# AbbVie-ComputationalGenomics/SAIGEgds

Measured on AMD Instinct MI355X. Metric: variants/sec seqAssocGLMM_SPA at N=430K; achieved HBM GB/s vs roofline, higher is better.
Workload: dtype f64

## Files before the change

saigegds_amd/csrc/host_init.h:

```cpp
extern "C" const char *sgx_version(void) { return "saigehip 0.1 (gfx950)"; }
extern "C" const char *sgx_last_error(void) { return g_err.c_str(); }

extern "C" int sgx_device_count(void)
{
	int n = 0;
	if (hipGetDeviceCount(&n) != hipSuccess) return 0;
	return n;
}

extern "C" size_t sgx_row_stride(int32_t n_samp)
{
	return (size_t)((n_samp + 511) / 512) * 128;
}

static double thr_or(double v, double dflt) { return std::isfinite(v) ? v : dflt; }

extern "C" int sgx_set_thresholds(sgx_handle *h, double maf, double mac, double missing,
	double spa_pval)
{
	if (!h) return fail(SGX_EINVAL, "sgx_set_thresholds: NULL handle");
	h->md.thr_maf = thr_or(maf, -1);
	h->md.thr_mac = thr_or(mac, -1);
	h->md.thr_missing = thr_or(missing, 1);
	h->md.thr_spa = thr_or(spa_pval, 0.05);
// ... 63 lines not shown
		}
	}
	if (!(worst <= 1e-13L * scale)) return false;
	for (int a = 0; a < K; a++)
		for (int b = 0; b < K; b++) out[(size_t)b * K + a] = (double)M[(size_t)a * K + b];
	for (int a = 0; a < K * K; a++) if (!std::isfinite(out[a])) return false;
	return true;
}

static int alloc_workspace(sgx_handle *h)
{
	const int N = h->md.N;
	{
		int least = 0, greatest = 0;
		HIPCHK(hipDeviceGetStreamPriorityRange(&least, &greatest));
		HIPCHK(hipStreamCreateWithPriority(&h->stream, hipStreamNonBlocking, least));
		HIPCHK(hipStreamCreateWithPriority(&h->hstream, hipStreamNonBlocking, greatest));
		HIPCHK(hipStreamCreateWithPriority(&h->s3_side, hipStreamNonBlocking, greatest));
	}
	HIPCHK(hipEventCreateWithFlags(&h->s3_fork, hipEventDisableTiming));
	HIPCHK(hipEventCreateWithFlags(&h->s3_join, hipEventDisableTiming));
	HIPCHK(hipMalloc((void **)&h->counters, 24 * sizeof(int)));
	HIPCHK(hipHostMalloc((void **)&h->h_counters, 24 * sizeof(int), hipHostMallocDefault));
	for (int i = 0; i < 3; i++) HIPCHK(hipEventCreate(&h->ev[i]));
	for (int i = 0; i < 2; i++) HIPCHK(hipEventCreate(&h->evk[i]));
	HIPCHK(hipEventCreate(&h->ev_lists));
	hipDeviceProp_t prop;
	HIPCHK(hipGetDeviceProperties(&prop, h->device));
	h->spa_grid = prop.multiProcessorCount * 2;
	h->n_cu = prop.multiProcessorCount;
	h->scratch_stride = 2 * (((size_t)N + 63) & ~(size_t)63);
	HIPCHK(hipMalloc((void **)&h->scratch, h->scratch_stride * sizeof(double) * h->spa_grid));
	if (!h->md.quant) {
		h->nwg5 = ((size_t)((N + 63) / 64) * 16 <= 32 * 1024) ? h->n_cu * 4 : h->n_cu;
		HIPCHK(hipMalloc((void **)&h->scr5, (size_t)h->nwg5 * spa5_wg_bytes(N)));
		HIPCHK(hipMalloc((void **)&h->cur5, 8 * sizeof(int)));
	}
	return SGX_OK;
}

static int check_model_consistency(const sgx_model *m)
{
	const int N = m->n_samp, K = m->n_coeff;
	if (!m->t_XXVX_inv || !m->XV)
		return fail(SGX_EINVAL, "sgx_init: SAIGEHIP_CHECK_MODEL needs t_XXVX_inv and XV");
	for (int i = 0; i < N; i++) {
		const double *x = m->t_X + (size_t)i * K, *xv = m->XV + (size_t)i * K,
			*a = m->t_XXVX_inv + (size_t)i * K, *av = m->t_XVX_inv_XV + (size_t)i * K;
		int k0 = 0;
		double sx = 0, sa = 0;
		for (int k = 0; k < K; k++) {
			if (std::fabs(x[k]) > std::fabs(x[k0])) k0 = k;
			sx = std::max(sx, std::fabs(xv[k])); sa = std::max(sa, std::fabs(av[k]));
		}
		if (x[k0] == 0) continue;
		const double V = xv[k0] / x[k0];
		for (int k = 0; k < K; k++) {
			if (std::fabs(xv[k] - V * x[k]) > 1e-8 * sx)
				return fail(SGX_EINVAL, "sgx_init: XV[%d,%d] = %g is not V t_X = %g", k, i, xv[k], V * x[k]);
			if (std::fabs(av[k] - V * a[k]) > 1e-8 * sa)
				return fail(SGX_EINVAL, "sgx_init: t_XVX_inv_XV[%d,%d] = %g is not V t_XXVX_inv = %g",
					k, i, av[k], V * a[k]);
		}
	}
	return SGX_OK;
}

extern "C" int sgx_init(const sgx_model *m, int device, sgx_handle **out)
// ... 155 lines not shown
		TRY(dev_upload(&h->dFl, Flu));
		h->mf[0].Fl = h->dFl;
		TRY(dev_upload(&h->dQ, Qt));
	}
	md.F = h->dF; md.X = h->dX; md.y = h->dy; md.mu = h->dmu; md.mu2 = h->dmu2; md.XM = h->dXM;
	rc = alloc_workspace(h);
	if (rc) { sgx_free(h); return rc; }
#undef TRY
	*out = h;
	return SGX_OK;
}

extern "C" int sgx_score_layout(sgx_handle *h, int32_t *limbs, int32_t n_limbs, int32_t *n_groups)
{
	if (!h || !n_groups) return fail(SGX_EINVAL, "sgx_score_layout: NULL argument");
	*n_groups = h->mf_ok ? h->mfe.ngroups : 0;
	for (int c = 0; limbs && c < n_limbs; c++) limbs[c] = (h->mf_ok && c < h->md.P) ? h->mfe.climb[c] : 0;
	return SGX_OK;
}

extern "C" void sgx_free(sgx_handle *h)
{
	if (!h) return;
	(void)hipSetDevice(h->device);
	if (h->stream) (void)hipStreamSynchronize(h->stream);
	for (sgx_handle *&t : h->twins) if (t) { sgx_free(t); t = nullptr; }
	if (!h->shares_model) {
		(void)hipFree(h->dF); (void)hipFree(h->dX); (void)hipFree(h->dy);
		(void)hipFree(h->dmu); (void)hipFree(h->dmu2); (void)hipFree(h->dXM); (void)hipFree(h->dFl); (void)hipFree(h->dQ);
	}
	(void)hipFree(h->fallback); (void)hipFree(h->fb_spa2); (void)hipFree(h->fb_x2);
	(void)hipFree(h->s3_slabs); (void)hipFree(h->s3_t3); (void)hipFree(h->s3_ovf);
	for (int b = 0; b < 2; b++) if (h->tmp_blk[b]) { sgx_block_free(h->tmp_blk[b]); h->tmp_blk[b] = nullptr; }
	(void)hipFree(h->mf_acc); (void)hipFree(h->seg4); (void)hipFree(h->scr5); (void)hipFree(h->cur5);
	(void)hipFree(h->recs); (void)hipFree(h->counters); (void)hipFree(h->scratch);
	for (int b = 0; b < 2; b++) {
		(void)hipFree(h->pipe_in[b]); (void)hipFree(h->pipe_pk[b]); (void)hipFree(h->pipe_raw[b]); (void)hipFree(h->pipe_out[b]); (void)hipFree(h->pipe_valid[b]);
		if (h->pin_out[b]) (void)hipHostFree(h->pin_out[b]);
		if (h->pin_valid[b]) (void)hipHostFree(h->pin_valid[b]);
	}
	(void)hipFree(h->pipe_flag); (void)hipFree(h->pk_sel);
	if (h->h_pipe_flag) (void)hipHostFree(h->h_pipe_flag);
	if (h->ev_h2d) (void)hipEventDestroy(h->ev_h2d);
	for (int k = 0; k < 2; k++) { if (h->ev_copy[k]) (void)hipEventDestroy(h->ev_copy[k]); if (h->ev_done[k]) (void)hipEventDestroy(h->ev_done[k]); }
	if (h->cstream) (void)hipStreamDestroy(h->cstream);
	(void)hipFree(h->stage_in); (void)hipFree(h->stage_out); (void)hipFree(h->stage_valid); (void)hipFree(h->stage_pk); (void)hipFree(h->ds_part);
	if (h->h_counters) (void)hipHostFree(h->h_counters);
	for (int i = 0; i < 3; i++) if (h->ev[i]) (void)hipEventDestroy(h->ev[i]);
	for (int i = 0; i < 2; i++) if (h->evk[i]) (void)hipEventDestroy(h->evk[i]);
	if (h->ev_lists) (void)hipEventDestroy(h->ev_lists);
	if (h->s3_side) { (void)hipStreamSynchronize(h->s3_side); (void)hipStreamDestroy(h->s3_side); }
	if (h->hstream) { (void)hipStreamSynchronize(h->hstream); (void)hipStreamDestroy(h->hstream); }
	if (h->s3_fork) (void)hipEventDestroy(h->s3_fork);
	if (h->s3_join) (void)hipEventDestroy(h->s3_join);
	if (h->stream) (void)hipStreamDestroy(h->stream);
	delete h;
}

static int ensure_recs(sgx_handle *h, size_t n)
{
	if (n <= h->recs_cap) return SGX_OK;
	HIPCHK(hipStreamSynchronize(h->stream));
	if (h->recs) HIPCHK(hipFree(h->recs));
	if (h->fallback) HIPCHK(hipFree(h->fallback));
	h->recs = nullptr; h->fallback = nullptr; h->recs_cap = 0;
	HIPCHK(hipMalloc((void **)&h->recs, 3 * n * sizeof(SpaRec)));
	HIPCHK(hipMalloc((void **)&h->fallback, n * sizeof(int)));
// ... 23 lines not shown
```

saigegds_amd/csrc/host_lanes.h:

```cpp
extern "C" int sgx_set_option(sgx_handle *h, const char *name, long long value)
{
	if (!h || !name) return fail(SGX_EINVAL, "sgx_set_option: NULL argument");
	const std::string n(name);
	if (n == "score_v1") h->force_v1 = value != 0;
	else if (n == "force_dense") h->force_dense = value != 0;
	else if (n == "spa_exact") h->force_exact = value != 0;
	else if (n == "pipe_mb") { if (value < 0 || value > 65536) return fail(SGX_EINVAL, "pipe_mb out of range"); h->pipe_bytes = (size_t)value << 20; return SGX_OK; }
	else if (n == "spa_abl") h->spa_abl = (int)value;
	else if (n == "guard_exp") { if (value < 0 || value > 300) return fail(SGX_EINVAL, "guard_exp must be 0..300"); h->guard_tol = std::pow(10.0, -(double)value); }
	else if (n == "three_plane") { if (value < -1 || value > 1) return fail(SGX_EINVAL, "three_plane must be -1 (automatic), 0 or 1"); h->dense_opt = (int)value; return SGX_OK; }
	else if (n == "lanes") {
		if (value < 1 || value > 4) return fail(SGX_EINVAL, "lanes must be 1..4");
		if (h->owner) return fail(SGX_EINVAL, "lanes: not on a twin");
		int rc = sgx_sync(h);
		if (rc) return rc;
		for (int i = (int)value - 1; i < 3; i++) if (h->twins[i]) { sgx_free(h->twins[i]); h->twins[i] = nullptr; }
		for (int i = 0; i < (int)value - 1; i++) {
			if (h->twins[i]) continue;
			sgx_handle *t = new sgx_handle();
			t->device = h->device; t->md = h->md; t->mf_ok = h->mf_ok; t->mfe = h->mfe;
			for (int g = 0; g < MF_MAXG; g++) { t->mf[g] = h->mf[g]; t->mf_nbfv[g] = h->mf_nbfv[g]; }
			t->dF = h->dF; t->dX = h->dX; t->dy = h->dy; t->dmu = h->dmu; t->dmu2 = h->dmu2; t->dXM = h->dXM; t->dFl = h->dFl; t->dQ = h->dQ;
			t->shares_model = true; t->owner = h;
			t->force_dense = h->force_dense; t->force_v1 = h->force_v1; t->force_exact = h->force_exact;
// ... 8 lines not shown
	}
	else return fail(SGX_EINVAL, "sgx_set_option: unknown option '%s'", name);
	for (sgx_handle *t : h->twins) if (t) { int rc = sgx_set_option(t, name, value); if (rc) return rc; }
	return SGX_OK;
}

static void stats_add(sgx_stats &into, const sgx_stats &x)
{
	into.n_variants += x.n_variants; into.n_valid += x.n_valid; into.n_spa += x.n_spa;
	into.n_spa_dense += x.n_spa_dense; into.n_spa_slow += x.n_spa_slow;
	into.ms_score += x.ms_score; into.ms_spa += x.ms_spa; into.ms_total += x.ms_total;
	into.ms_kernel += x.ms_kernel; into.ms_lists += x.ms_lists;
	into.score_launches += x.score_launches; into.spa_launches += x.spa_launches;
	into.three_plane += x.three_plane; into.n_unlisted += x.n_unlisted; into.n_guarded += x.n_guarded;
}

static int sync_lane(sgx_handle *h)
{
	int rc = set_dev(h);
	if (rc) return rc;
	HIPCHK(hipStreamSynchronize(h->stream));
	if (h->pend_dense.active) {
		h->pend_dense.active = false;
		if (h->stats_pending && h->h_counters[2] > 0) {
			rc = launch_pending_dense(h);
			if (rc) return rc;
			HIPCHK(hipStreamSynchronize(h->stream));
		}
	}
	if (h->stats_pending) {
		h->stats.n_spa = (uint64_t)(h->h_counters[0] + h->h_counters[7] - h->h_counters[6] + h->h_counters[5]);
		h->stats.n_valid = (uint64_t)h->h_counters[1];
		h->stats.n_spa_dense = (uint64_t)h->h_counters[2];
		h->stats.n_spa_slow = (uint64_t)h->h_counters[4];
		h->stats.three_plane = h->form == FORM_THREE ? 1u : 0u;
		h->stats.n_guarded = (uint32_t)h->h_counters[21];
		h->stats.n_unlisted = (uint32_t)h->h_counters[23] - h->stats.n_guarded;
		if (h->form != FORM_FP64) {
			sgx_handle *p = h->owner ? h->owner : h;
			const double frac = 64.0 * (double)h->h_counters[22] / ((double)std::max<uint64_t>(1, h->stats.n_variants) * (double)h->md.N);
			const bool over = (uint64_t)h->stats.n_unlisted * 32 > h->stats.n_variants;
			if (h->form != FORM_THREE && (frac > SGX_DENSE_ON || over)) p->dense_mode = true;
			else if (h->form == FORM_THREE && frac < SGX_DENSE_OFF) p->dense_mode = false;
		}
#ifdef SPA5_PROF
		fprintf(stderr, "routing: tier A %d, tier B %d (of them handed on by A: %d), per-variant kernels %d (series list %d, exact list %d), dense %d\n",
			h->h_counters[0], h->h_counters[7], h->h_counters[6], h->h_counters[5], h->h_counters[3], h->h_counters[4], h->h_counters[2]);
		fprintf(stderr, "spa5 phases (10 ns ticks summed over variants): series kernel %d variants: stage %d count %d index %d gather %d series %d (sweep %d sum %d solve %d) | exact kernel %d variants: stage %d count %d index %d gather %d - sweeps %d\n",
			h->h_counters[3], h->h_counters[8], h->h_counters[9], h->h_counters[10], h->h_counters[11], h->h_counters[12], h->h_counters[13], h->h_counters[14], h->h_counters[15],
			h->h_counters[4], h->h_counters[16], h->h_counters[17], h->h_counters[18], h->h_counters[19], h->h_counters[21]);
#endif
		float a = 0, b = 0, c = 0;
		(void)hipEventElapsedTime(&a, h->ev[0], h->ev[1]);
		(void)hipEventElapsedTime(&b, h->ev[1], h->ev[2]);
		(void)hipEventElapsedTime(&c, h->ev[0], h->ev[2]);
		h->stats.ms_score = a; h->stats.ms_spa = b; h->stats.ms_total = c;
		float k = 0;
		if (h->evk_set) (void)hipEventElapsedTime(&k, h->evk[0], h->evk[1]);
		h->stats.ms_kernel = k; h->evk_set = false;
		float l = 0;
		if (h->lists_timed) { (void)hipEventElapsedTime(&l, h->ev_lists, h->ev[0]); h->stats.ms_total += l; }
		h->stats.ms_lists = l; h->lists_timed = false;
		h->stats_pending = false;
		sgx_handle *p = h->owner ? h->owner : h;
		stats_add(p->total, h->stats);
		p->total_calls++;
	}
// ... 31 lines not shown
```

saigegds_amd/csrc/host_spa.h:

```cpp


template <int LO, typename F, int... I>
static bool with_int(int v, F &&f, std::integer_sequence<int, I...>)
{
	return ((v == LO + I && (f(std::integral_constant<int, LO + I>()), true)) || ...);
}
template <typename F>
static bool with_k(int K, F &&f) { return with_int<1>(K, f, std::make_integer_sequence<int, KMAX>()); }
template <typename F>
static void with_pp(int P, F &&f)
{
	if (P <= 8) f(std::integral_constant<int, 8>());
	else if (P <= 16) f(std::integral_constant<int, 16>());
	else if (P <= 32) f(std::integral_constant<int, 32>());
	else f(std::integral_constant<int, 64>());
}

static dim3 mf_grid(int n_cu, size_t rows, int ntile, int *tps, int vpb = MF_VPB, int wg_per_cu = 2)
{
	const int vt = (int)((rows + vpb - 1) / vpb);
	int sk = std::max(1, (n_cu * wg_per_cu * 4 + vt / 2) / vt);
	sk = std::min(sk, std::max(1, ntile / 24));
	if (sk >= 6) sk = (sk + 7) & ~7;
	sk = std::min(sk, std::max(1, ntile / 2));
// ... 1 lines not shown
	*tps += *tps & 1;
	sk = (ntile + *tps - 1) / *tps;
	return dim3((unsigned)vt, (unsigned)sk);
}

template <int KK, int NCX, int INPUT>
static const void *spa4_moments_fn()
{
	if constexpr (INPUT == IN_2BIT) return (const void *)spa4_moments<KK, NCX>;
	else return (const void *)spa4_moments_ds<KK, NCX, INPUT>;
}

template <int KK, int INPUT>
static int launch_spa_k(sgx_handle *h, RowsRef rr, size_t M, double *out8, bool lazy_dense)
{
	const DevModel &md = h->md;
	constexpr int PB = 512;
	hipStream_t st = h->stream;
	const dim3 sgrid((unsigned)std::min<size_t>(M, (size_t)h->spa_grid));
	if (h->force_v1 && INPUT != IN_2BIT) {
		hipLaunchKernelGGL((spa_kernel<KK, PB, INPUT>), sgrid, dim3(PB), 0, st, rr,
			md, h->recs, h->counters, 0, (const int *)nullptr, h->scratch, h->scratch_stride, out8);
		return SGX_OK;
	}
	const size_t fl = spa4_lds_bytes(KK);
	if (!h->mom_attr_set[INPUT]) {
		HIPCHK(hipFuncSetAttribute(spa4_moments_fn<KK, SPA4_NCA, INPUT>(), hipFuncAttributeMaxDynamicSharedMemorySize, (int)fl));
		HIPCHK(hipFuncSetAttribute(spa4_moments_fn<KK, SPA4_NCB, INPUT>(), hipFuncAttributeMaxDynamicSharedMemorySize, (int)fl));
		h->mom_attr_set[INPUT] = true;
	}
	const int nround = (int)((M + h->vcap4 - 1) / h->vcap4);
	const int btop = (int)(2 * M);
	const dim3 gsolve((unsigned)std::min((h->vcap4 + 3) / 4, 4 * h->n_cu));
	const size_t rowb5 = (size_t)((md.N + 63) / 64) * 16;
	const size_t l5 = (INPUT == IN_2BIT && rowb5 <= 120 * 1024) ? rowb5 : 0;
	const bool small5 = INPUT == IN_2BIT && rowb5 <= 32 * 1024;
	if (l5 > 48 * 1024 && !h->spa5_attr_set[INPUT]) {
		HIPCHK(hipFuncSetAttribute((const void *)spa5_kernel<KK, INPUT, 0, 512>, hipFuncAttributeMaxDynamicSharedMemorySize, (int)l5));
		HIPCHK(hipFuncSetAttribute((const void *)spa5_kernel<KK, INPUT, 1, 512>, hipFuncAttributeMaxDynamicSharedMemorySize, (int)l5));
		h->spa5_attr_set[INPUT] = true;
	}
	const int fx5 = (h->force_exact ? 1 : 0) | (h->spa_abl & ~1);
	auto moments = [&](auto ncx, int tier, int rd) {
		constexpr int NCX = decltype(ncx)::value;
		if constexpr (INPUT == IN_2BIT)
			hipLaunchKernelGGL((spa4_moments<KK, NCX>), dim3((unsigned)h->n_cu), dim3(WAVE * spa4_waves(KK)), fl, st, rr, md, h->nseg,
				tier, btop, rd * h->vcap4, h->vcap4, h->recs, h->counters, h->seg4, h->spa_abl, h->cur5 + 2);
		else
			hipLaunchKernelGGL((spa4_moments_ds<KK, NCX, INPUT>), dim3((unsigned)h->n_cu), dim3(WAVE * spa4_waves(KK)), fl, st,
				(const void *)rr.base, rr.bpv, md, h->nseg, tier, btop, rd * h->vcap4, h->vcap4, h->recs, h->counters, h->seg4, h->cur5 + 2);
		hipLaunchKernelGGL((spa4_solve<KK, NCX>), gsolve, dim3(256), 0, st, md, h->nseg, tier, btop, rd * h->vcap4, h->vcap4,
			h->recs, h->counters, h->seg4, h->fallback, h->fb_x2, out8, h->force_dense ? 1 : 0, h->force_exact ? 1 : 0);
	};
	for (int rd = 0; rd < nround; rd++) moments(std::integral_constant<int, SPA4_NCA>(), 0, rd);
	for (int rd = 0; rd < nround; rd++) moments(std::integral_constant<int, SPA4_NCB>(), 1, rd);
	const int only5 = (INPUT == IN_2BIT && rr.cptr != nullptr && (h->spa_abl & 512)) ? 2 : 0;
	const size_t ws5 = spa5_wg_bytes(md.N);
	auto spa5 = [&](auto threads, int nwg) {
		constexpr int T5 = decltype(threads)::value;
		if constexpr (T5 == 512 || INPUT == IN_2BIT) {
			hipLaunchKernelGGL((spa5_kernel<KK, INPUT, 0, T5>), dim3((unsigned)nwg), dim3(T5), l5, st, rr, md, h->recs, h->counters,
				h->fb_spa2, h->fb_x2, h->cur5, h->fallback, h->scr5, out8, h->force_dense ? 1 : 0, fx5, l5, only5, ws5, 3);
			hipLaunchKernelGGL((spa5_kernel<KK, INPUT, 1, T5>), dim3((unsigned)nwg), dim3(T5), l5, st, rr, md, h->recs, h->counters,
				h->fb_x2, h->fb_x2, h->cur5 + 1, h->fallback, h->scr5, out8, h->force_dense ? 1 : 0, fx5, l5, only5, ws5, 4);
		}
	};
	if (small5) spa5(std::integral_constant<int, 128>(), h->nwg5);
	else spa5(std::integral_constant<int, 512>(), h->n_cu);
	if (!lazy_dense)
		hipLaunchKernelGGL((spa_kernel<KK, PB, INPUT>), sgrid, dim3(PB), 0, st, rr,
			md, h->recs, h->counters, 2, h->fallback, h->scratch, h->scratch_stride, out8);
	return SGX_OK;
}

template <int INPUT>
static int launch_spa(sgx_handle *h, RowsRef rr, size_t M, double *out8, bool lazy_dense = false)
{
	h->stats.spa_launches = 0;
	if (h->md.quant) return SGX_OK;
	int rc = SGX_OK;
	with_k(h->md.K, [&](auto kk) { rc = launch_spa_k<decltype(kk)::value, INPUT>(h, rr, M, out8, lazy_dense); });
	if (rc) return rc;
	HIPCHK(hipGetLastError());
	const bool v1 = h->force_v1 && INPUT != IN_2BIT;
	h->stats.spa_launches = v1 ? 1u : (uint32_t)(4 * ((M + h->vcap4 - 1) / h->vcap4) + 3);
	if (lazy_dense && !v1) { h->pend_dense.active = true; h->pend_dense.rr = rr; h->pend_dense.M = M; h->pend_dense.out8 = out8; }
	return SGX_OK;
}

static int launch_pending_dense(sgx_handle *h)
{
	const dim3 sgrid((unsigned)std::min<size_t>(h->pend_dense.M, (size_t)h->spa_grid));
	with_k(h->md.K, [&](auto kk) {
		hipLaunchKernelGGL((spa_kernel<decltype(kk)::value, 512, IN_2BIT>), sgrid, dim3(512), 0, h->stream, h->pend_dense.rr, h->md,
			h->recs, h->counters, 2, h->fallback, h->scratch, h->scratch_stride, h->pend_dense.out8);
	});
	HIPCHK(hipGetLastError());
	return SGX_OK;
}

static int scan_begin(sgx_handle *h, hipStream_t sst, ScanForm form, const sgx_block *b)
// ... 84 lines not shown
```

saigegds_amd/csrc/host_state.h:

```cpp

struct sgx_block {
	int device = 0;
	int N = 0, ntile = 0, nr = 1;
	size_t cap = 0;
	size_t M = 0;
	bool lists_only = false;
	uint8_t *rows = nullptr;
	size_t bpv = 0;
	const uint8_t *ext_rows = nullptr; size_t ext_bpv = 0;
	unsigned *idx = nullptr; size_t idx_cap = 0;
	unsigned *cursor = nullptr;
	unsigned *lstart = nullptr;
	int *lcnt = nullptr;
	int *nzp = nullptr, *n2p = nullptr;
	int *n3 = nullptr;
	uint8_t *ovf = nullptr;
	int *nzv = nullptr, *n2v = nullptr;
	unsigned *cptr = nullptr;
	unsigned *cidx = nullptr;
	size_t cidx_cap = 0;
	uint8_t *corient = nullptr;
	hipEvent_t ready = nullptr;
	hipEvent_t last_read = nullptr;
	bool was_read = false;
	int *info = nullptr, *h_info = nullptr;
	bool info_read = false, dense = false;
};

enum ScanForm {
	FORM_FP64,
	FORM_LISTS,
	FORM_ROWS,
	FORM_THREE,
};

struct sgx_handle {
	int device = 0;
	hipStream_t stream = nullptr;
	DevModel md{};
	double *dF = nullptr, *dX = nullptr, *dy = nullptr, *dmu = nullptr, *dmu2 = nullptr, *dXM = nullptr;
	SpaRec *recs = nullptr; size_t recs_cap = 0;
	int *fallback = nullptr;
	int *fb_spa2 = nullptr;
	int *fb_x2 = nullptr;
	int nseg = 0;
	bool force_dense = false;
	double *seg4 = nullptr;
	int vcap4 = 0, nround4 = 0;
	bool spa5_attr_set[3] = {false, false, false};
	bool mom_attr_set[3] = {false, false, false};
	uint8_t *scr5 = nullptr; int *cur5 = nullptr; int nwg5 = 0;
	int spa_abl = 0;
	bool force_exact = false;
	bool mf_ok = false;
	MfTab mf[MF_MAXG]{};
	int mf_nbfv[MF_MAXG]{};
	MfEpi mfe{};
	uint8_t *dFl = nullptr;
	long long *dQ = nullptr;
	int *mf_acc = nullptr;
	int *s3_slabs = nullptr; size_t s3_slabs_cap = 0;
	long long *s3_t3 = nullptr; size_t s3_t3_cap = 0;
	int *s3_ovf = nullptr; size_t s3_ovf_cap = 0;
	bool s3_attr[17] = {false};
	bool s3_attr_miss[17] = {false};
	hipStream_t hstream = nullptr;
	hipStream_t s3_side = nullptr;
	hipEvent_t s3_fork = nullptr, s3_join = nullptr;
	sgx_block *tmp_blk[2] = {nullptr, nullptr};
	int n_cu = 256;
	int *counters = nullptr;
	int *h_counters = nullptr;
	double *scratch = nullptr; size_t scratch_stride = 0; int spa_grid = 0;
	uint8_t *stage_in = nullptr; size_t stage_in_cap = 0;
	hipStream_t cstream = nullptr;
	size_t pipe_bytes = 0;
	uint8_t *pipe_in[2] = {nullptr, nullptr}; size_t pipe_in_cap = 0;
	uint8_t *pipe_pk[2] = {nullptr, nullptr}; size_t pipe_pk_cap = 0;
	uint8_t *pipe_raw[2] = {nullptr, nullptr}; size_t pipe_raw_cap = 0;
	int *pk_sel = nullptr; size_t pk_sel_cap = 0;
	double *pipe_out[2] = {nullptr, nullptr}; uint8_t *pipe_valid[2] = {nullptr, nullptr}; size_t pipe_out_cap = 0;
	double *pin_out[2] = {nullptr, nullptr}; uint8_t *pin_valid[2] = {nullptr, nullptr};
	int *pipe_flag = nullptr, *h_pipe_flag = nullptr;
	hipEvent_t ev_h2d = nullptr;
// ... 36 lines not shown
```

saigegds_amd/csrc/kern_spa4.h:

```cpp
#pragma once
#include "kern_spa4_tab.h"


#ifndef SPA4_WAVES_LOWK
#define SPA4_WAVES_LOWK 8
#endif
__host__ __device__ constexpr int spa4_waves(int K) { return K <= 8 ? SPA4_WAVES_LOWK : 8; }
#define SPA4_NCA 12
#define SPA4_NCB SPA4_NC
#define SPA4_NSMAX (SPA4_NC + 5)
#define SPA4_TAIL_TOL 1e-10

__device__ __forceinline__ double spa4_fma_svv(double a_sgpr, double x, double c_vgpr)
{
	double r;
	asm("v_fma_f64 %0, %1, %2, %3" : "=v"(r) : "s"(a_sgpr), "v"(x), "v"(c_vgpr));
	return r;
}

__device__ __forceinline__ void spa4_max_abs(double &g, double a)
{
	asm("v_max_f64 %0, %0, |%1|" : "+v"(g) : "v"(a));
}

// ... 508 lines not shown
			recs[btop - 1 - slot] = r;
		} else {
			fb_exact[atomicAdd(&counters[4], 1)] = ri;
		}
		return;
	}
	double pval;
	bool converged = true;
	if ((st_mine & 2) && (st_other & 2)) {
		pval = fabs(p_mine) + fabs(p_other);
		if (pval != 0 && pn_in / pval > 1000) pval = pn_in;
	} else {
		pval = pn_in;
		converged = false;
	}
	spa_write_row(r, Tstat, var1, pval, converged, out8);
}


#define SPA5_BIG 2048

__device__ __forceinline__ void cgf_terms_rt(double g, double m, double t, bool with_k, double &k1, double &k2, double &k0)
{
	const double om = 1 - m, mg = m * g, c2 = om * mg * g;
	const double e = fast_exp(-g * t);
	const double d = fma(om, e, m);
	const double rr = isfinite(d) ? fast_rcp(d) : 0.0;
	k1 = fma(mg, rr, k1);
	const double tt = c2 * e * rr * rr;
	if (isfinite(tt)) k2 += tt;
	if (with_k) k0 += cgf_korg_term(g, m, t, d, om);
}

__host__ __device__ inline size_t spa5_wg_bytes(int N) { return (((size_t)N + 63) & ~(size_t)63) * (16 + 4); }

template <int BLOCK>
__device__ __noinline__ void spa5_cum_sweep(const double2 *__restrict__ glist, int nnz, double ts, double *kp_out)
{
	constexpr int NC = SPA4_NCB;
	double kp[NC - 1];
#pragma unroll
	for (int a = 0; a < NC - 1; a++) kp[a] = 0;
	double2 gn = (int)threadIdx.x < nnz ? glist[threadIdx.x] : make_double2(0.0, 0.5);
	for (int k = threadIdx.x; k < nnz; k += BLOCK) {
		const double2 gm = gn;
		if (k + BLOCK < nnz) gn = glist[k + BLOCK];
		const double mui = gm.y;
		spa4_cum_terms<NC>(gm.x * ts, mui * (1 - mui), 1 - 2 * mui, kp);
		kp[NC - 2] = fmax(kp[NC - 2], fabs(gm.x));
	}
#pragma unroll
	for (int a = 0; a < NC - 1; a++) kp_out[a] = kp[a];
}

__device__ __noinline__ int spa5_series_solve(const double *arg, const SpaRec *__restrict__ rec, double *__restrict__ out8)
{
	constexpr int NC = SPA4_NCB;
	Spa4Series<NC> S;
#pragma unroll
	for (int a = 0; a < NC - 2; a++) S.kp[a] = arg[a];
	S.k1 = arg[NC - 2]; S.k2 = arg[NC - 1]; S.ts = arg[NC]; S.gmax = arg[NC + 1];
	const double xmax = arg[NC + 2], qtilde = arg[NC + 3], qinv = arg[NC + 4], NAmu = arg[NC + 5], NAsigma = arg[NC + 6];
	const double pn_in = arg[NC + 7], Tstat = arg[NC + 8], var1 = arg[NC + 9];
	RootState s1, s2;
	if (!spa4_root(S, xmax, qtilde, NAmu, NAsigma, s1) || !spa4_root(S, xmax, qinv, NAmu, NAsigma, s2)) return 0;
	double pval;
	bool converged = true;
// ... 31 lines not shown
	const int lane = threadIdx.x & (WAVE - 1), wv = threadIdx.x / WAVE;
	double kr[NC - 2];
#pragma unroll
	for (int a = 0; a < NC - 2; a++) kr[a] = kp[a];
	const int idx = wave_reduce_scatter(kr, lane);
#pragma unroll
	for (int o = 32; o > 0; o >>= 1) gmax = fmax(gmax, __shfl_xor(gmax, o, WAVE));
	double *part = sh + NC + 16;
	if (!(lane & 3) && idx < NC - 2) part[idx * NWV + wv] = kr[0];
	if (lane == 1) part[(NC - 2) * NWV + wv] = gmax;
	__syncthreads();
	double *arg = sh;
	if (threadIdx.x < NC - 2) {
		double t = 0;
		for (int w = 0; w < NWV; w++) t += part[threadIdx.x * NWV + w];
		arg[threadIdx.x] = t;
	}
	__syncthreads();
	SPA5_TS(1);
	if (threadIdx.x == 0) {
		for (int w = 0; w < NWV; w++) gmax = fmax(gmax, part[(NC - 2) * NWV + w]);
		arg[NC - 2] = k1; arg[NC - 1] = k2; arg[NC] = ts; arg[NC + 1] = gmax; arg[NC + 2] = xmax;
		arg[NC + 3] = qtilde; arg[NC + 4] = qinv; arg[NC + 5] = NAmu; arg[NC + 6] = NAsigma;
		arg[NC + 7] = pn_in; arg[NC + 8] = Tstat; arg[NC + 9] = var1;
		*sh_flag = spa5_series_solve(arg, rec, out8);
	}
	SPA5_TS(2);
	__syncthreads();
	const bool done = *sh_flag != 0;
	__syncthreads();
	return done;
}

#ifndef SPA5_REG_WAVES
#define SPA5_REG_WAVES 2
#endif
#define SPA5_WAVES_PER_SIMD(BLOCK) ((BLOCK) == 512 ? SPA5_REG_WAVES : ((BLOCK) / 64 + 3) / 4)
#ifdef SPA5_PROF
#define SPA5_T(ph) do { if (tid == 0) { const long long now_ = wall_clock64(); atomicAdd(&counters[8 + 8 * MODE + (ph)], (int)(now_ - tprev_)); tprev_ = now_; } } while (0)
#else
#define SPA5_T(ph) do { } while (0)
#endif
template <int K, int INPUT, int MODE, int BLOCK>
__global__ void __launch_bounds__(BLOCK, SPA5_WAVES_PER_SIMD(BLOCK))
spa5_kernel(RowsRef rr, DevModel md, const SpaRec *__restrict__ recs,
	int *__restrict__ counters, const int *__restrict__ todo, int *__restrict__ todo_next, int *__restrict__ cursor,
	int *__restrict__ fb_dense, uint8_t *__restrict__ scratch, double *__restrict__ out8, int force_dense, int force_exact,
	size_t lds_row_bytes, int only, size_t wg_stride, int nslot)
{
	constexpr int KP = (K + 2) & ~1, NW = BLOCK / WAVE;
	extern __shared__ __attribute__((aligned(16))) uint8_t fill_smem[];
	uint4 *rows_lds = reinterpret_cast<uint4 *>(fill_smem);
	__shared__ double sh[SPA4_NCB * NW + SPA4_NCB + 16];
	__shared__ int sh_flag;
	__shared__ int shi[NW];
	__shared__ int sh_vi, sh_v;
	__shared__ SpaRec sh_rec;
	const int N = md.N, tid = threadIdx.x, lane = tid & (WAVE - 1), wid = tid / WAVE;
	double2 *glist = reinterpret_cast<double2 *>(scratch + (size_t)blockIdx.x * wg_stride);
	uint32_t *ilist = reinterpret_cast<uint32_t *>(glist + (((size_t)N + 63) & ~(size_t)63));
	const int ntodo = counters[nslot];
	const int nvec = INPUT == IN_2BIT ? (int)(min((size_t)((N + 63) >> 6) * 16, rr_row_bytes(rr)) / 16) : (N + 63) >> 6;
	const int per = ((nvec + NW - 1) / NW + WAVE - 1) & ~(WAVE - 1);
	for (;;) {
		__syncthreads();
		if (tid < WAVE) {
			int vi0 = 0;
			if (tid == 0) vi0 = atomicAdd(cursor, 1);
			vi0 = __builtin_amdgcn_readfirstlane(vi0);
			int v0 = -1;
			if (vi0 < 2 * ntodo) {
				v0 = todo[vi0 < ntodo ? vi0 : vi0 - ntodo];
				const double *src = reinterpret_cast<const double *>(recs + v0);
				for (int i = tid; i < (int)(sizeof(SpaRec) / 8); i += WAVE) reinterpret_cast<double *>(&sh_rec)[i] = src[i];
			}
			if (tid == 0) { sh_vi = vi0; sh_v = v0; }
		}
		__syncthreads();
		const int vi = sh_vi;
		if (vi >= 2 * ntodo) break;
#ifdef SPA5_PROF
		long long tprev_ = wall_clock64();
#endif
		const bool big_round = vi < ntodo;
		const int v = sh_v;
		const SpaRec &r = sh_rec;
		if ((r.nnz > SPA5_BIG) != big_round) continue;
		auto row_piece = [&](int p) -> uint4 { return *reinterpret_cast<const uint4 *>(rr.base + rr_piece(rr, (size_t)r.j, (size_t)p)); };
		const uint32_t zx = r.minus ? 0xAAAAAAAAu : 0u;
		const double lut0 = r.lut[0], lut1 = r.lut[1], lut2 = r.lut[2], lut3 = r.lut[3];
		const bool listed = INPUT == IN_2BIT && only != 2 && rr.cptr != nullptr && rr.corient[r.j] == (r.minus ? 2 : 1);
		const uint32_t *il = listed ? rr.cidx + rr.cptr[r.j] : ilist;
		int nnz = listed ? r.nnz : 0;
		if (!listed) {
			const bool staged = INPUT == IN_2BIT && lds_row_bytes >= (size_t)nvec * 16;
			if (staged) {
				constexpr int UN = 8;
				for (int p0 = tid; p0 < nvec; p0 += UN * BLOCK) {
					uint4 t[UN];
	#pragma unroll
					for (int j = 0; j < UN; j++) { const int p = p0 + j * BLOCK; t[j] = p < nvec ? row_piece(p) : make_uint4(0u, 0u, 0u, 0u); }
	#pragma unroll
					for (int j = 0; j < UN; j++) { const int p = p0 + j * BLOCK; if (p < nvec) rows_lds[p] = t[j]; }
				}
				__syncthreads();
			}
			SPA5_T(0);
			auto masks = [&](int p, uint32_t (&ww)[4], uint32_t (&z)[4]) -> int {
				int cnt = 0;
				if (INPUT == IN_2BIT) {
					uint4 w = make_uint4(0u, 0u, 0u, 0u);
					if (p < nvec) w = staged ? rows_lds[p] : row_piece(p);
					ww[0] = w.x; ww[1] = w.y; ww[2] = w.z; ww[3] = w.w;
	#pragma unroll
					for (int k = 0; k < 4; k++) { z[k] = nz_fields((ww[k] ^ zx) & keep_mask(N - p * 64 - 16 * k)); cnt += __popc(z[k]); }
				} else {
					z[0] = z[1] = z[2] = z[3] = 0;
					if (p < nvec) {
						for (int s2 = 0; s2 < 64; s2++) {
							const int i = p * 64 + s2;
							if (i < N && load_dosage<INPUT>(rr, i, r) != 0) { z[s2 >> 5] |= 1u << (s2 & 31); cnt++; }
						}
					}
				}
				return cnt;
			};
			int cnt_w = 0;
			for (int it = 0; it < per; it += WAVE) {
				uint32_t ww[4], z[4];
				cnt_w += masks(wid * per + it + lane, ww, z);
			}
			cnt_w = wave_sum_i(cnt_w);
			if (lane == 0) shi[wid] = cnt_w;
			__syncthreads();
			int o_w = 0;
	#pragma unroll
			for (int w = 0; w < NW; w++) { if (w < wid) o_w += shi[w]; nnz += shi[w]; }
			SPA5_T(1);
			for (int it = 0; it < per; it += WAVE) {
				uint32_t ww[4], z[4];
				const int p = wid * per + it + lane;
				const int cnt = masks(p, ww, z);
				if (!__ballot(cnt != 0)) continue;
				int incl = cnt;
	#pragma unroll
				for (int o = 1; o < WAVE; o <<= 1) {
					const int up = __shfl_up(incl, o, WAVE);
					if (lane >= o) incl += up;
				}
				int o2 = o_w + incl - cnt;
				o_w += __shfl(incl, WAVE - 1, WAVE);
				if (INPUT == IN_2BIT) {
	#pragma unroll
					for (int k = 0; k < 4; k++) {
						uint32_t zz = z[k];
						while (zz) {
							const int b = __ffs(zz) - 1;
							zz &= zz - 1;
							ilist[o2++] = (uint32_t)(p * 64 + 16 * k + (b >> 1)) | (((ww[k] >> b) & 3u) << 30);
						}
					}
				} else {
	#pragma unroll
					for (int k = 0; k < 2; k++) {
						uint32_t zz = z[k];
						while (zz) {
							const int b = __ffs(zz) - 1;
							zz &= zz - 1;
							ilist[o2++] = (uint32_t)(p * 64 + 32 * k + b);
						}
					}
				}
			}
			__syncthreads();
			SPA5_T(2);
		}
		const double inv = 1 / sqrt(r.AC2);
		double c[K];
#pragma unroll
		for (int a = 0; a < K; a++) c[a] = r.c[a];
		double a6[6] = {0, 0, 0, 0, 0, 0};
		constexpr int UNG = K <= 4 ? 4 : 2;
		for (int k0 = tid; k0 < ((force_exact & 128) ? 0 : nnz); k0 += UNG * BLOCK) {
			uint32_t e[UNG];
			double xv[UNG][KP];
#pragma unroll
			for (int j = 0; j < UNG; j++) e[j] = (k0 + j * BLOCK < nnz) ? il[k0 + j * BLOCK] : 0u;
#pragma unroll
			for (int j = 0; j < UNG; j++) {
				const double *x = md.XM + (size_t)(e[j] & 0x3FFFFFFFu) * KP;
#pragma unroll
				for (int a = 0; a < KP; a += 2) {
					const double2 t2 = *reinterpret_cast<const double2 *>(x + a);
					xv[j][a] = t2.x; xv[j][a + 1] = t2.y;
				}
			}
#pragma unroll
			for (int j = 0; j < UNG; j++) {
				const int k = k0 + j * BLOCK;
				if (k >= nnz) continue;
				const uint32_t code = e[j] >> 30;
				const double G = INPUT == IN_2BIT ? ((code & 2u) ? ((code & 1u) ? lut3 : lut2) : ((code & 1u) ? lut1 : lut0))
// ... 6 lines not shown
				glist[k] = make_double2(adj, mui);
				a6[0] = fma(mui, G, a6[0]);
				a6[1] += b;
				if (adj > 0) a6[2] += adj; else a6[3] += adj;
				a6[4] = fma(adj, mui, a6[4]);
				a6[5] = fma(adj * adj, mui * (1 - mui), a6[5]);
			}
		}
		block_sum<6, BLOCK>(a6, sh);
		SPA5_T(3);
		double xmu_c = 0, xsum_c = 0;
#pragma unroll
		for (int a = 0; a < K; a++) { xmu_c = fma(md.Xmu[a], c[a], xmu_c); xsum_c = fma(md.Xsum[a], c[a], xsum_c); }
		const double m1 = (a6[0] - xmu_c) * inv;
		const double Tstat = r.S * inv;
		const double var2 = r.var2 / r.AC2, var1 = var2 * md.r;
		const double qtilde = Tstat / sqrt(var1) * sqrt(var2) + m1;
		const double sdev = qtilde - m1, qinv = -sdev + m1;
		const double pn_in = d_pchisq1_upper(sdev * sdev / var2);
		double pval;
		bool converged = true;
		if (fabs(qtilde - m1) / sqrt(var2) < 2.0) {
			pval = pn_in;
		} else {
			const double nb = (xsum_c - a6[1]) * inv;
			const double L = a6[2] + fmax(-nb, 0.0), U = a6[3] + fmin(-nb, 0.0);
			const double mar = 1e-9 * (fabs(L) + fabs(U) + fabs(qtilde) + fabs(qinv));
			if (force_dense || !(qtilde < L - mar && qtilde > U + mar && qinv < L - mar && qinv > U + mar)) {
				if (tid == 0) fb_dense[atomicAdd(&counters[2], 1)] = v;
				continue;
			}
			const double NAmu = m1 - a6[4], NAsigma = var2 - a6[5];
			if (MODE == 0) {
				if ((force_exact & 1) || !spa5_series<BLOCK>(glist, nnz, r.tscale, md.spa_xmax, a6[4], a6[5], qtilde, qinv, NAmu, NAsigma,
						pn_in, Tstat, var1, &sh_rec, out8, sh, &sh_flag, counters + 13)) {
					if (tid == 0) todo_next[atomicAdd(&counters[4], 1)] = v;
				}
				SPA5_T(4);
				continue;
			}
			RootState s1, s2;
			root_begin(s1, qtilde, L, U);
			root_begin(s2, qinv, L, U);
			root_feed(s1, a6[4], a6[5], NAmu, NAsigma, 0.0, true);
			root_feed(s2, a6[4], a6[5], NAmu, NAsigma, 0.0, true);
			auto sweep = [&](bool a1, bool a2, bool k1w, bool k2w, double t1, double t2, double (&sv)[6]) {
#pragma unroll
				for (int a = 0; a < 6; a++) sv[a] = 0;
				double2 gn = tid < nnz ? glist[tid] : make_double2(0.0, 0.5);
				for (int k0 = tid; k0 < nnz; k0 += BLOCK) {
					const double2 gm = gn;
					if (k0 + BLOCK < nnz) gn = glist[k0 + BLOCK];
					if (a1) cgf_terms_rt(gm.x, gm.y, t1, k1w, sv[0], sv[1], sv[2]);
					if (a2) cgf_terms_rt(gm.x, gm.y, t2, k2w, sv[3], sv[4], sv[5]);
				}
				block_sum<6, BLOCK>(sv, sh);
			};
			while ((s1.active || s2.active) && !(force_exact & 64)) {
				const bool a1 = s1.active, a2 = s2.active, k1w = s1.want_k, k2w = s2.want_k;
				double sv[6];
				sweep(a1, a2, k1w, k2w, s1.tnew, s2.tnew, sv);
				if (a1) root_feed(s1, sv[0], sv[1], NAmu, NAsigma, sv[2], k1w);
				if (a2) root_feed(s2, sv[3], sv[4], NAmu, NAsigma, sv[5], k2w);
			}
			if (s1.converged && s2.converged) {
				if (!(s1.k_ok && s2.k_ok)) {
					double sv[6];
					sweep(!s1.k_ok, !s2.k_ok, true, true, s1.root, s2.root, sv);
					if (!s1.k_ok) s1.Kcur = sv[2];
					if (!s2.k_ok) s2.Kcur = sv[5];
				}
				const double p1 = lugannani_rice(s1.root, s1.Kcur, s1.K2cur, qtilde, NAmu, NAsigma);
// ... 13 lines not shown
```

Before: 18.28 million.

## Restructure SPA5 kernel: drop LDS row staging, split small/big scratch, inline slow path

Removes the dynamic-LDS row staging in spa5_kernel and instead register-batches 8 global row-piece loads per wave, allowing smaller blocks (256 threads, 2 WGs/CU) with higher occupancy. Scratch is split into capped per-WG small buffers plus a few full-size big buffers reserved for high-nnz variants, cutting scratch footprint; variants exceeding the small cap fall back to the dense path. MODE 0 no longer defers series failures to a todo_next list but falls through into the root-finding path in the same kernel, counted via a new counter. It risks more dense fallbacks and different load scheduling without LDS reuse across the two mask passes.

```diff
diff --git a/saigegds_amd/csrc/host_init.h b/saigegds_amd/csrc/host_init.h
--- a/saigegds_amd/csrc/host_init.h
+++ b/saigegds_amd/csrc/host_init.h
@@ -119,8 +119,10 @@
 	h->scratch_stride = 2 * (((size_t)N + 63) & ~(size_t)63);
 	HIPCHK(hipMalloc((void **)&h->scratch, h->scratch_stride * sizeof(double) * h->spa_grid));
 	if (!h->md.quant) {
-		h->nwg5 = ((size_t)((N + 63) / 64) * 16 <= 32 * 1024) ? h->n_cu * 4 : h->n_cu;
-		HIPCHK(hipMalloc((void **)&h->scr5, (size_t)h->nwg5 * spa5_wg_bytes(N)));
+		h->nwg5 = h->n_cu * SPA5_WG_PER_CU;
+		HIPCHK(hipMalloc((void **)&h->scr5, (size_t)h->nwg5 * spa5_wg_bytes(spa5_small_cap(N))));
+		h->nbig5 = spa5_big_cap(N) > spa5_small_cap(N) ? h->n_cu : 0;
+		if (h->nbig5) HIPCHK(hipMalloc((void **)&h->scr5_big, (size_t)h->nbig5 * spa5_wg_bytes(spa5_big_cap(N))));
 		HIPCHK(hipMalloc((void **)&h->cur5, 8 * sizeof(int)));
 	}
 	return SGX_OK;
@@ -342,7 +344,7 @@
 	(void)hipFree(h->fallback); (void)hipFree(h->fb_spa2); (void)hipFree(h->fb_x2);
 	(void)hipFree(h->s3_slabs); (void)hipFree(h->s3_t3); (void)hipFree(h->s3_ovf);
 	for (int b = 0; b < 2; b++) if (h->tmp_blk[b]) { sgx_block_free(h->tmp_blk[b]); h->tmp_blk[b] = nullptr; }
-	(void)hipFree(h->mf_acc); (void)hipFree(h->seg4); (void)hipFree(h->scr5); (void)hipFree(h->cur5);
+	(void)hipFree(h->mf_acc); (void)hipFree(h->seg4); (void)hipFree(h->scr5); (void)hipFree(h->scr5_big); (void)hipFree(h->cur5);
 	(void)hipFree(h->recs); (void)hipFree(h->counters); (void)hipFree(h->scratch);
 	for (int b = 0; b < 2; b++) {
 		(void)hipFree(h->pipe_in[b]); (void)hipFree(h->pipe_pk[b]); (void)hipFree(h->pipe_raw[b]); (void)hipFree(h->pipe_out[b]); (void)hipFree(h->pipe_valid[b]);
diff --git a/saigegds_amd/csrc/host_lanes.h b/saigegds_amd/csrc/host_lanes.h
--- a/saigegds_amd/csrc/host_lanes.h
+++ b/saigegds_amd/csrc/host_lanes.h
@@ -64,7 +64,7 @@
 		h->stats.n_spa = (uint64_t)(h->h_counters[0] + h->h_counters[7] - h->h_counters[6] + h->h_counters[5]);
 		h->stats.n_valid = (uint64_t)h->h_counters[1];
 		h->stats.n_spa_dense = (uint64_t)h->h_counters[2];
-		h->stats.n_spa_slow = (uint64_t)h->h_counters[4];
+		h->stats.n_spa_slow = (uint64_t)(h->h_counters[4] + h->h_counters[20]);
 		h->stats.three_plane = h->form == FORM_THREE ? 1u : 0u;
 		h->stats.n_guarded = (uint32_t)h->h_counters[21];
 		h->stats.n_unlisted = (uint32_t)h->h_counters[23] - h->stats.n_guarded;
diff --git a/saigegds_amd/csrc/host_spa.h b/saigegds_amd/csrc/host_spa.h
--- a/saigegds_amd/csrc/host_spa.h
+++ b/saigegds_amd/csrc/host_spa.h
@@ -57,14 +57,7 @@
 	const int nround = (int)((M + h->vcap4 - 1) / h->vcap4);
 	const int btop = (int)(2 * M);
 	const dim3 gsolve((unsigned)std::min((h->vcap4 + 3) / 4, 4 * h->n_cu));
-	const size_t rowb5 = (size_t)((md.N + 63) / 64) * 16;
-	const size_t l5 = (INPUT == IN_2BIT && rowb5 <= 120 * 1024) ? rowb5 : 0;
-	const bool small5 = INPUT == IN_2BIT && rowb5 <= 32 * 1024;
-	if (l5 > 48 * 1024 && !h->spa5_attr_set[INPUT]) {
-		HIPCHK(hipFuncSetAttribute((const void *)spa5_kernel<KK, INPUT, 0, 512>, hipFuncAttributeMaxDynamicSharedMemorySize, (int)l5));
-		HIPCHK(hipFuncSetAttribute((const void *)spa5_kernel<KK, INPUT, 1, 512>, hipFuncAttributeMaxDynamicSharedMemorySize, (int)l5));
-		h->spa5_attr_set[INPUT] = true;
-	}
+	const bool small5 = INPUT == IN_2BIT && (size_t)((md.N + 63) / 64) * 16 <= 32 * 1024;
 	const int fx5 = (h->force_exact ? 1 : 0) | (h->spa_abl & ~1);
 	auto moments = [&](auto ncx, int tier, int rd) {
 		constexpr int NCX = decltype(ncx)::value;
@@ -80,18 +73,17 @@
 	for (int rd = 0; rd < nround; rd++) moments(std::integral_constant<int, SPA4_NCA>(), 0, rd);
 	for (int rd = 0; rd < nround; rd++) moments(std::integral_constant<int, SPA4_NCB>(), 1, rd);
 	const int only5 = (INPUT == IN_2BIT && rr.cptr != nullptr && (h->spa_abl & 512)) ? 2 : 0;
-	const size_t ws5 = spa5_wg_bytes(md.N);
-	auto spa5 = [&](auto threads, int nwg) {
+	auto spa5 = [&](auto threads) {
 		constexpr int T5 = decltype(threads)::value;
-		if constexpr (T5 == 512 || INPUT == IN_2BIT) {
-			hipLaunchKernelGGL((spa5_kernel<KK, INPUT, 0, T5>), dim3((unsigned)nwg), dim3(T5), l5, st, rr, md, h->recs, h->counters,
-				h->fb_spa2, h->fb_x2, h->cur5, h->fallback, h->scr5, out8, h->force_dense ? 1 : 0, fx5, l5, only5, ws5, 3);
-			hipLaunchKernelGGL((spa5_kernel<KK, INPUT, 1, T5>), dim3((unsigned)nwg), dim3(T5), l5, st, rr, md, h->recs, h->counters,
-				h->fb_x2, h->fb_x2, h->cur5 + 1, h->fallback, h->scr5, out8, h->force_dense ? 1 : 0, fx5, l5, only5, ws5, 4);
+		if constexpr (T5 == SPA5_BLOCK_L || INPUT == IN_2BIT) {
+			hipLaunchKernelGGL((spa5_kernel<KK, INPUT, 0, T5>), dim3((unsigned)h->nwg5), dim3(T5), 0, st, rr, md, h->recs, h->counters,
+				h->fb_spa2, h->cur5, h->fallback, h->scr5, h->scr5_big, 0, out8, h->force_dense ? 1 : 0, fx5, only5, 3);
+			hipLaunchKernelGGL((spa5_kernel<KK, INPUT, 1, T5>), dim3((unsigned)h->nwg5), dim3(T5), 0, st, rr, md, h->recs, h->counters,
+				h->fb_x2, h->cur5 + 1, h->fallback, h->scr5, h->scr5_big, h->nbig5, out8, h->force_dense ? 1 : 0, fx5, only5, 4);
 		}
 	};
-	if (small5) spa5(std::integral_constant<int, 128>(), h->nwg5);
-	else spa5(std::integral_constant<int, 512>(), h->n_cu);
+	if (small5) spa5(std::integral_constant<int, 128>());
+	else spa5(std::integral_constant<int, SPA5_BLOCK_L>());
 	if (!lazy_dense)
 		hipLaunchKernelGGL((spa_kernel<KK, PB, INPUT>), sgrid, dim3(PB), 0, st, rr,
 			md, h->recs, h->counters, 2, h->fallback, h->scratch, h->scratch_stride, out8);
diff --git a/saigegds_amd/csrc/host_state.h b/saigegds_amd/csrc/host_state.h
--- a/saigegds_amd/csrc/host_state.h
+++ b/saigegds_amd/csrc/host_state.h
@@ -47,9 +47,9 @@
 	bool force_dense = false;
 	double *seg4 = nullptr;
 	int vcap4 = 0, nround4 = 0;
-	bool spa5_attr_set[3] = {false, false, false};
 	bool mom_attr_set[3] = {false, false, false};
 	uint8_t *scr5 = nullptr; int *cur5 = nullptr; int nwg5 = 0;
+	uint8_t *scr5_big = nullptr; int nbig5 = 0;
 	int spa_abl = 0;
 	bool force_exact = false;
 	bool mf_ok = false;
diff --git a/saigegds_amd/csrc/kern_spa4.h b/saigegds_amd/csrc/kern_spa4.h
--- a/saigegds_amd/csrc/kern_spa4.h
+++ b/saigegds_amd/csrc/kern_spa4.h
@@ -564,7 +564,9 @@
 	if (with_k) k0 += cgf_korg_term(g, m, t, d, om);
 }
 
-__host__ __device__ inline size_t spa5_wg_bytes(int N) { return (((size_t)N + 63) & ~(size_t)63) * (16 + 4); }
+__host__ __device__ inline size_t spa5_big_cap(int N) { return ((size_t)N + 63) & ~(size_t)63; }
+__host__ __device__ inline size_t spa5_small_cap(int N) { return spa5_big_cap(N) < (size_t)SPA5_NNZ ? spa5_big_cap(N) : (size_t)SPA5_NNZ; }
+__host__ __device__ inline size_t spa5_wg_bytes(size_t cap) { return cap * (16 + 4); }
 
 template <int BLOCK>
 __device__ __noinline__ void spa5_cum_sweep(const double2 *__restrict__ glist, int nnz, double ts, double *kp_out)
@@ -662,10 +664,13 @@
 	return done;
 }
 
-#ifndef SPA5_REG_WAVES
-#define SPA5_REG_WAVES 2
+#ifndef SPA5_BLOCK_L
+#define SPA5_BLOCK_L 256
 #endif
-#define SPA5_WAVES_PER_SIMD(BLOCK) ((BLOCK) == 512 ? SPA5_REG_WAVES : ((BLOCK) / 64 + 3) / 4)
+#ifndef SPA5_WG_PER_CU
+#define SPA5_WG_PER_CU 2
+#endif
+#define SPA5_WAVES_PER_SIMD(BLOCK) ((BLOCK) == SPA5_BLOCK_L ? ((BLOCK) / 64 * SPA5_WG_PER_CU + 3) / 4 : ((BLOCK) / 64 + 3) / 4)
 #ifdef SPA5_PROF
 #define SPA5_T(ph) do { if (tid == 0) { const long long now_ = wall_clock64(); atomicAdd(&counters[8 + 8 * MODE + (ph)], (int)(now_ - tprev_)); tprev_ = now_; } } while (0)
 #else
@@ -674,30 +679,37 @@
 template <int K, int INPUT, int MODE, int BLOCK>
 __global__ void __launch_bounds__(BLOCK, SPA5_WAVES_PER_SIMD(BLOCK))
 spa5_kernel(RowsRef rr, DevModel md, const SpaRec *__restrict__ recs,
-	int *__restrict__ counters, const int *__restrict__ todo, int *__restrict__ todo_next, int *__restrict__ cursor,
-	int *__restrict__ fb_dense, uint8_t *__restrict__ scratch, double *__restrict__ out8, int force_dense, int force_exact,
-	size_t lds_row_bytes, int only, size_t wg_stride, int nslot)
+	int *__restrict__ counters, const int *__restrict__ todo, int *__restrict__ cursor,
+	int *__restrict__ fb_dense, uint8_t *__restrict__ scratch, uint8_t *__restrict__ scratch_big, int nbig,
+	double *__restrict__ out8, int force_dense, int force_exact, int only, int nslot)
 {
 	constexpr int KP = (K + 2) & ~1, NW = BLOCK / WAVE;
-	extern __shared__ __attribute__((aligned(16))) uint8_t fill_smem[];
-	uint4 *rows_lds = reinterpret_cast<uint4 *>(fill_smem);
 	__shared__ double sh[SPA4_NCB * NW + SPA4_NCB + 16];
 	__shared__ int sh_flag;
 	__shared__ int shi[NW];
 	__shared__ int sh_vi, sh_v;
 	__shared__ SpaRec sh_rec;
 	const int N = md.N, tid = threadIdx.x, lane = tid & (WAVE - 1), wid = tid / WAVE;
-	double2 *glist = reinterpret_cast<double2 *>(scratch + (size_t)blockIdx.x * wg_stride);
-	uint32_t *ilist = reinterpret_cast<uint32_t *>(glist + (((size_t)N + 63) & ~(size_t)63));
+	const bool has_big = MODE == 1 && (int)blockIdx.x < nbig;
+	const int small_cap = (int)spa5_small_cap(N);
+	const int cap = has_big ? (int)spa5_big_cap(N) : small_cap;
+	double2 *glist = reinterpret_cast<double2 *>(has_big ? scratch_big + (size_t)blockIdx.x * spa5_wg_bytes(spa5_big_cap(N))
+		: scratch + (size_t)blockIdx.x * spa5_wg_bytes((size_t)small_cap));
+	uint32_t *ilist = reinterpret_cast<uint32_t *>(glist + cap);
 	const int ntodo = counters[nslot];
 	const int nvec = INPUT == IN_2BIT ? (int)(min((size_t)((N + 63) >> 6) * 16, rr_row_bytes(rr)) / 16) : (N + 63) >> 6;
 	const int per = ((nvec + NW - 1) / NW + WAVE - 1) & ~(WAVE - 1);
+	int hpos = has_big ? (int)blockIdx.x : ntodo;
 	for (;;) {
 		__syncthreads();
+		const bool big_slot_round = hpos < ntodo;
 		if (tid < WAVE) {
 			int vi0 = 0;
-			if (tid == 0) vi0 = atomicAdd(cursor, 1);
-			vi0 = __builtin_amdgcn_readfirstlane(vi0);
+			if (big_slot_round) vi0 = hpos;
+			else {
+				if (tid == 0) vi0 = atomicAdd(cursor, 1);
+				vi0 = __builtin_amdgcn_readfirstlane(vi0);
+			}
 			int v0 = -1;
 			if (vi0 < 2 * ntodo) {
 				v0 = todo[vi0 < ntodo ? vi0 : vi0 - ntodo];
@@ -706,6 +718,7 @@
 			}
 			if (tid == 0) { sh_vi = vi0; sh_v = v0; }
 		}
+		if (big_slot_round) hpos += nbig;
 		__syncthreads();
 		const int vi = sh_vi;
 		if (vi >= 2 * ntodo) break;
@@ -715,7 +728,15 @@
 		const bool big_round = vi < ntodo;
 		const int v = sh_v;
 		const SpaRec &r = sh_rec;
-		if ((r.nnz > SPA5_BIG) != big_round) continue;
+		if (big_slot_round) {
+			if (r.nnz <= small_cap) continue;
+		} else {
+			if (r.nnz > small_cap) {
+				if (MODE == 0 && big_round && tid == 0) fb_dense[atomicAdd(&counters[2], 1)] = v;
+				continue;
+			}
+			if ((r.nnz > SPA5_BIG) != big_round) continue;
+		}
 		auto row_piece = [&](int p) -> uint4 { return *reinterpret_cast<const uint4 *>(rr.base + rr_piece(rr, (size_t)r.j, (size_t)p)); };
 		const uint32_t zx = r.minus ? 0xAAAAAAAAu : 0u;
 		const double lut0 = r.lut[0], lut1 = r.lut[1], lut2 = r.lut[2], lut3 = r.lut[3];
@@ -723,24 +744,17 @@
 		const uint32_t *il = listed ? rr.cidx + rr.cptr[r.j] : ilist;
 		int nnz = listed ? r.nnz : 0;
 		if (!listed) {
-			const bool staged = INPUT == IN_2BIT && lds_row_bytes >= (size_t)nvec * 16;
-			if (staged) {
-				constexpr int UN = 8;
-				for (int p0 = tid; p0 < nvec; p0 += UN * BLOCK) {
-					uint4 t[UN];
-	#pragma unroll
-					for (int j = 0; j < UN; j++) { const int p = p0 + j * BLOCK; t[j] = p < nvec ? row_piece(p) : make_uint4(0u, 0u, 0u, 0u); }
-	#pragma unroll
-					for (int j = 0; j < UN; j++) { const int p = p0 + j * BLOCK; if (p < nvec) rows_lds[p] = t[j]; }
-				}
-				__syncthreads();
-			}
-			SPA5_T(0);
-			auto masks = [&](int p, uint32_t (&ww)[4], uint32_t (&z)[4]) -> int {
+			constexpr int UN = INPUT == IN_2BIT ? 8 : 1;
+			auto load_pieces = [&](int it, uint4 (&t)[UN]) {
+#pragma unroll
+				for (int j = 0; j < UN; j++) {
+					const int p = wid * per + it + j * WAVE + lane;
+					t[j] = (INPUT == IN_2BIT && it + j * WAVE < per && p < nvec) ? row_piece(p) : make_uint4(0u, 0u, 0u, 0u);
+				}
+			};
+			auto masks = [&](int p, const uint4 &w, uint32_t (&ww)[4], uint32_t (&z)[4]) -> int {
 				int cnt = 0;
 				if (INPUT == IN_2BIT) {
-					uint4 w = make_uint4(0u, 0u, 0u, 0u);
-					if (p < nvec) w = staged ? rows_lds[p] : row_piece(p);
 					ww[0] = w.x; ww[1] = w.y; ww[2] = w.z; ww[3] = w.w;
 	#pragma unroll
 					for (int k = 0; k < 4; k++) { z[k] = nz_fields((ww[k] ^ zx) & keep_mask(N - p * 64 - 16 * k)); cnt += __popc(z[k]); }
@@ -756,9 +770,14 @@
 				return cnt;
 			};
 			int cnt_w = 0;
-			for (int it = 0; it < per; it += WAVE) {
-				uint32_t ww[4], z[4];
-				cnt_w += masks(wid * per + it + lane, ww, z);
+			for (int it = 0; it < per; it += UN * WAVE) {
+				uint4 t[UN];
+				load_pieces(it, t);
+	#pragma unroll
+				for (int j = 0; j < UN; j++) {
+					uint32_t ww[4], z[4];
+					if (it + j * WAVE < per) cnt_w += masks(wid * per + it + j * WAVE + lane, t[j], ww, z);
+				}
 			}
 			cnt_w = wave_sum_i(cnt_w);
 			if (lane == 0) shi[wid] = cnt_w;
@@ -767,37 +786,47 @@
 	#pragma unroll
 			for (int w = 0; w < NW; w++) { if (w < wid) o_w += shi[w]; nnz += shi[w]; }
 			SPA5_T(1);
-			for (int it = 0; it < per; it += WAVE) {
-				uint32_t ww[4], z[4];
-				const int p = wid * per + it + lane;
-				const int cnt = masks(p, ww, z);
-				if (!__ballot(cnt != 0)) continue;
-				int incl = cnt;
+			if (nnz > cap) {
+				if (tid == 0) fb_dense[atomicAdd(&counters[2], 1)] = v;
+				continue;
+			}
+			for (int it = 0; it < per; it += UN * WAVE) {
+				uint4 t[UN];
+				load_pieces(it, t);
 	#pragma unroll
-				for (int o = 1; o < WAVE; o <<= 1) {
-					const int up = __shfl_up(incl, o, WAVE);
-					if (lane >= o) incl += up;
-				}
-				int o2 = o_w + incl - cnt;
-				o_w += __shfl(incl, WAVE - 1, WAVE);
-				if (INPUT == IN_2BIT) {
+				for (int j = 0; j < UN; j++) {
+					if (it + j * WAVE >= per) continue;
+					uint32_t ww[4], z[4];
+					const int p = wid * per + it + j * WAVE + lane;
+					const int cnt = masks(p, t[j], ww, z);
+					if (!__ballot(cnt != 0)) continue;
+					int incl = cnt;
 	#pragma unroll
-					for (int k = 0; k < 4; k++) {
-						uint32_t zz = z[k];
-						while (zz) {
-							const int b = __ffs(zz) - 1;
-							zz &= zz - 1;
-							ilist[o2++] = (uint32_t)(p * 64 + 16 * k + (b >> 1)) | (((ww[k] >> b) & 3u) << 30);
+					for (int o = 1; o < WAVE; o <<= 1) {
+						const int up = __shfl_up(incl, o, WAVE);
+						if (lane >= o) incl += up;
+					}
+					int o2 = o_w + incl - cnt;
+					o_w += __shfl(incl, WAVE - 1, WAVE);
+					if (INPUT == IN_2BIT) {
+	#pragma unroll
+						for (int k = 0; k < 4; k++) {
+							uint32_t zz = z[k];
+							while (zz) {
+								const int b = __ffs(zz) - 1;
+								zz &= zz - 1;
+								ilist[o2++] = (uint32_t)(p * 64 + 16 * k + (b >> 1)) | (((ww[k] >> b) & 3u) << 30);
+							}
 						}
-					}
-				} else {
+					} else {
 	#pragma unroll
-					for (int k = 0; k < 2; k++) {
-						uint32_t zz = z[k];
-						while (zz) {
-							const int b = __ffs(zz) - 1;
-							zz &= zz - 1;
-							ilist[o2++] = (uint32_t)(p * 64 + 32 * k + b);
+						for (int k = 0; k < 2; k++) {
+							uint32_t zz = z[k];
+							while (zz) {
+								const int b = __ffs(zz) - 1;
+								zz &= zz - 1;
+								ilist[o2++] = (uint32_t)(p * 64 + 32 * k + b);
+							}
 						}
 					}
 				}
@@ -870,12 +899,13 @@
 			}
 			const double NAmu = m1 - a6[4], NAsigma = var2 - a6[5];
 			if (MODE == 0) {
-				if ((force_exact & 1) || !spa5_series<BLOCK>(glist, nnz, r.tscale, md.spa_xmax, a6[4], a6[5], qtilde, qinv, NAmu, NAsigma,
+				if (!(force_exact & 1) && spa5_series<BLOCK>(glist, nnz, r.tscale, md.spa_xmax, a6[4], a6[5], qtilde, qinv, NAmu, NAsigma,
 						pn_in, Tstat, var1, &sh_rec, out8, sh, &sh_flag, counters + 13)) {
-					if (tid == 0) todo_next[atomicAdd(&counters[4], 1)] = v;
-				}
+					SPA5_T(4);
+					continue;
+				}
+				if (tid == 0) atomicAdd(&counters[20], 1);
 				SPA5_T(4);
-				continue;
 			}
 			RootState s1, s2;
 			root_begin(s1, qtilde, L, U);
```

Measured after the change: 17.52 million. -4.2%, worse.
